# wiedenhoeft/HaMMLET

Hardware: AMD Instinct MI355X
Metric: block-updates/sec (Gibbs sweep) + HBM GB/s, 10^8 pos / 5 states (higher is better)
Workload: dtype f32; 1 GPU; c3_1e8_k5_dynamic; positions=100000000, states=5, block_structure=dynamic, chains=1, parallelism=chain-parallel x1

## Files before the change

hammlet_amd/csrc/hml_capi.hip:

```cpp
#include "hml_capi_shared.hpp"

static thread_local std::string g_err;
int hml_set_err(int code, const std::string& msg) { g_err = msg; return code; }

static const hml_ktab* ktab(int K);
#define HML_KTAB(KV, tab) const hml_ktab* tab = ktab(KV); if (!tab) return set_err(HML_ERR_ARG, "number of states must be in [2,16]")

std::atomic<int> hml_live_ctx[64];
int hml_ctx_bind(hml_ctx* c) { return ctx_bind(c); }
int hml_ctx_fetch_model(hml_ctx* c, hml_model* out) { return fetch_model(c, out); }

HML_KERNEL void hml_k_debug_eval(int fn, const float* __restrict__ a, const float* __restrict__ b, float* __restrict__ out,
                                 uint64_t n, uint64_t seed) {
    if (fn == 24) {
        const uint64_t nw = ((uint64_t)gridDim.x * blockDim.x) >> 6;
        if ((threadIdx.x & 63) != 0) return;
        for (uint64_t i = ((uint64_t)blockIdx.x * blockDim.x + threadIdx.x) >> 6; i < n; i += nw) {
            hml_dev_src src;
            src.s = hml_stream_open(hml_make_key(seed, 0), HML_KIND_THETA, seed, (uint32_t)i);
            out[i] = hml_gamma_f32<hml_devmath>(src, a[i], b[i]);
        }
        return;
    }
    const uint64_t stride = (uint64_t)gridDim.x * blockDim.x;
    for (uint64_t i = (uint64_t)blockIdx.x * blockDim.x + threadIdx.x; i < n; i += stride) {
        const float x = a[i], y = b ? b[i] : 0.0f;
        float r = 0.0f;
        switch (fn) {
            case 0: r = hml_expf(x); break;
            case 1: r = hml_logf(x); break;
            case 2: r = hml_powf_unit(x, y); break;
            case 3: r = HML_SQRTF(x); break;
            case 4: r = x / y; break;
            case 5: {
                hml_dev_src src;
                src.s = hml_stream_open(hml_make_key(seed, 0), HML_KIND_THETA, seed, (uint32_t)i);
                r = hml_gamma_f32<hml_devmath>(src, x, y);
            } break;
            case 6: {
                hml_dev_src src;
                src.s = hml_stream_open(hml_make_key(seed, 0), HML_KIND_PI, seed, (uint32_t)i);
                hml_normal_f32<hml_devmath> nd;
                r = nd.draw(src, x, y);
            } break;
            case 7: r = (float)hml_log((double)x); break;
            case 8: r = (float)hml_exp_nonpos((double)x); break;
            case 9: r = (float)((double)x / (double)y); break;
            case 40: r = hml_glibc_expf(x); break;
            case 41: r = hml_glibc_logf(x); break;
            case 42: r = hml_glibc_powf_unit(x, y); break;
            case 43: { const double Zd = (double)y; r = hml_tr2_quotient(x, Zd, hml_tr2_reciprocal(Zd)); } break;
            case 10: r = (float)(1.0 / (double)x); break;
            case 12: case 13: case 14: case 15: case 16: case 17: case 18: case 19: case 20: case 21: case 22: case 23: {
                hml_dev_src src; src.s = hml_stream_open(hml_make_key(seed, 0), HML_KIND_THETA, seed, (uint32_t)i);
                const float alpha = x, beta = y; (void)beta;
                const float malpha = alpha < 1.0f ? alpha + 1.0f : alpha;
                const float a1 = malpha - 1.0f / 3.0f;
                const float a2 = 1.0f / hml_devmath::sqrtf_(9.0f * a1);
                hml_normal_f32<hml_devmath> nd;
                float n = nd.draw(src, 0.0f, 1.0f);
                float v = 1.0f + a2 * n;
                float v3 = v * v * v;
                float u = hml_canonical_f32(src);
                const bool c1 = (double)u > (double)1.0f - 0.0331 * (double)n * (double)n * (double)n * (double)n;
                const bool c2 = ((double)hml_devmath::logf_(u) > (0.5 * (double)n * (double)n + (double)a1 * ((1.0 - (double)v3) + (double)hml_devmath::logf_(v3))));
                float n2 = nd.draw(src, 0.0f, 1.0f);
                float vb = 1.0f + a2 * n2;
                float vb3 = vb * vb * vb;
                float ub = hml_canonical_f32(src);
                const bool d1 = (double)ub > (double)1.0f - 0.0331 * (double)n2 * (double)n2 * (double)n2 * (double)n2;
                const bool d2 = ((double)hml_devmath::logf_(ub) > (0.5 * (double)n2 * (double)n2 + (double)a1 * ((1.0 - (double)vb3) + (double)hml_devmath::logf_(vb3))));
                r = fn == 12 ? n : fn == 13 ? v3 : fn == 14 ? u : fn == 15 ? (float)(c1 ? 1 : 0) + 2.0f * (c2 ? 1 : 0) : fn == 16 ? n2 : fn == 17 ? a2
                    : fn == 18 ? vb3 : fn == 19 ? ub : fn == 20 ? (float)(d1 ? 1 : 0) + 2.0f * (d2 ? 1 : 0) : fn == 21 ? (float)src.s.n : 0.0f;
                if (fn == 22) r = nd.draw(src, 0.0f, 1.0f);
                if (fn == 23) { hml_normal_f32<hml_devmath> nf; r = nf.draw(src, 0.0f, 1.0f); r = nf.draw(src, 0.0f, 1.0f); }
            } break;
            case 30: case 31: {
                r = 0.0f;
                const int Kc = fn == 30 ? 16 : 5;
                if (i % Kc == 0 && i + Kc <= n) {
                    bool unsure = false;
                    int fastr, lit;
                    if (fn == 30) { float w[16]; for (int j = 0; j < 16; ++j) w[j] = a[i + j]; fastr = hml_categorical_k_fast<16>(w, (double)y, unsure); lit = hml_categorical_k_literal<16>(w, (double)y); if (unsure) fastr = lit; }
                    else { float w[5]; for (int j = 0; j < 5; ++j) w[j] = a[i + j]; fastr = hml_categorical_k_fast<5>(w, (double)y, unsure); lit = hml_categorical_k_literal<5>(w, (double)y); if (unsure) fastr = lit; }
                    out[i] = (float)fastr; out[i + 1] = (float)lit; out[i + 2] = unsure ? 1.0f : 0.0f;
                }
                continue;
            }
            case 11: { const double d = HML_SQRT((double)x * 1.0000001); r = (float)((d - (double)(float)d) * 1e9); } break;
        }
        out[i] = r;
    }
}

static bool parse_band_edges(const char* text, int* n, float* edges) {
    *n = 0;
    const char* p = text;
    while (*p) {
        char* end = nullptr;
        const float v = strtof(p, &end);
        if (end == p || *n >= HML_MAX_BAND_EDGES) return false;
        edges[(*n)++] = v;
        p = end;
// ... 1121 lines not shown
        for (int k = 0; k < n; ++k) {
            hml_ctx* c = cs[k];
            if (int r = ctx_bind(c)) return r;
            if (record && c->rec_marginals && c->pooled) return set_err(HML_ERR_ARG, "the marginals of a context are pooled (common labels, several chains): further sweeps cannot be recorded into them");
            if (chain_halted(c)) { if (int r = hml_settle(c)) return r; }
            log_sweep(c, method, record);
            if (int r = sweep_dispatch(c, method, record)) return r;
            if (record && c->cb) {
                HIPCHK(hipStreamSynchronize(c->stream));
                if (chain_halted(c)) { if (int r = hml_settle(c)) return r; continue; }
                if (int r = check_device_error(c)) return r;
                c->cb(c, i, c->cb_user);
            }
        }
    }
    return 0;
}

extern "C" {

int hml_set_option(hml_ctx* c, const char* name, int value) {
    if (!c || !name) return set_err(HML_ERR_ARG, "null argument");
    if (std::string(name) == "weight_keys") {
        if (c->loaded) return set_err(HML_ERR_ARG, "weight_keys must be set before the observations are loaded");
        c->use_keys = value != 0;
        c->summary_always = value == 2;
        return 0;
    }
    if (std::string(name) == "max_blocks") {
        if (c->loaded) return set_err(HML_ERR_ARG, "max_blocks must be set before the observations are loaded");
        if (value < 0) return set_err(HML_ERR_ARG, "max_blocks: a number of blocks, or 0 for the default");
        c->cap_opt = (uint64_t)value;
        return 0;
    }
    if (std::string(name) == "fused_blocks") {
        c->fused_blocks = value != 0;
        c->fused_keep = value == 2;
        if (c->graph_exec) { hipGraphExecDestroy(c->graph_exec); c->graph_exec = nullptr; }
        return 0;
    }
    if (std::string(name) == "compat") {
        if (c->model_set) return set_err(HML_ERR_ARG, "compat must be set before the model");
        c->compat = value != 0;
        return 0;
    }
    if (std::string(name) == "trellis_L") {
        if (value < 0 || value > HML_TRE_MAX_L || value % 32) return set_err(HML_ERR_ARG, "trellis_L: 0 or a multiple of 32 up to 1024");
        c->tre_L = (uint32_t)value;
        return 0;
    }
    return set_err(HML_ERR_ARG, std::string("unknown option ") + name);
}

int hml_sync(hml_ctx* c) {
    if (!c) return set_err(HML_ERR_ARG, "null context");
    if (int r = ctx_bind(c)) return r;
    if (int r = hml_settle(c)) return r;
    if (c->d_dbg && getenv("HML_FUSED_DEBUG") && atoi(getenv("HML_FUSED_DEBUG")) == 2) {
        std::vector<unsigned long long> h(4096 * 8);
        hipMemcpy(h.data(), c->d_dbg, h.size() * 8, hipMemcpyDeviceToHost);
        uint32_t n = 0; while (n < 4096 && h[n * 8]) ++n;
        unsigned long long t0 = ~0ull; for (uint32_t i = 0; i < n; ++i) t0 = std::min(t0, h[i * 8]);
        double mx[5] = {0, 0, 0, 0, 0}, av[5] = {0, 0, 0, 0, 0};
        if (n) for (uint32_t i = 0; i < n; ++i) for (int k = 0; k < 5; ++k) { const double d = (double)(h[i * 8 + k] - t0) * 0.01; mx[k] = std::max(mx[k], d); av[k] += d / n; }
        if (n) fprintf(stderr, "[fused-many dbg] n=%u start avg %.2f max %.2f | phaseA avg %.2f max %.2f | requested avg %.2f max %.2f | offsets avg %.2f max %.2f | end avg %.2f max %.2f (us)\n",
                n, av[0], mx[0], av[1], mx[1], av[2], mx[2], av[3], mx[3], av[4], mx[4]);
        if (n) for (uint32_t i : {0u, n / 4, n / 2, n - 1}) if (i < n) fprintf(stderr, "   wg %u: %.2f %.2f %.2f %.2f %.2f | wavefront 0: parameters in LDS %.2f, weights arrived %.2f, its lists done %.2f\n", i, (h[i*8]-t0)*0.01, (h[i*8+1]-t0)*0.01, (h[i*8+2]-t0)*0.01, (h[i*8+3]-t0)*0.01, (h[i*8+4]-t0)*0.01,
                                                                                  (h[i*8+5]-t0)*0.01, (h[i*8+6]-t0)*0.01, (h[i*8+7]-t0)*0.01);
    } else if (c->d_dbg) {
        std::vector<unsigned long long> h(4096 * 4);
        hipMemcpy(h.data(), c->d_dbg, h.size() * 8, hipMemcpyDeviceToHost);
        const uint32_t n = (uint32_t)std::min<uint64_t>(4096, (c->T + HML_FUSED_SUB_POSITIONS - 1) / HML_FUSED_SUB_POSITIONS);
        unsigned long long t0 = ~0ull; for (uint32_t i = 0; i < n; ++i) if (h[i * 4]) t0 = std::min(t0, h[i * 4]);
        double mx[4] = {0, 0, 0, 0}, av[4] = {0, 0, 0, 0};
        for (uint32_t i = 0; i < n; ++i) for (int k = 0; k < 4; ++k) { const double d = (double)(h[i * 4 + k] - t0) * 0.01; mx[k] = std::max(mx[k], d); av[k] += d / n; }
        fprintf(stderr, "[fused dbg] n=%u start avg %.2f max %.2f | phaseA avg %.2f max %.2f | offsets avg %.2f max %.2f | end avg %.2f max %.2f (us)\n", n, av[0], mx[0], av[1], mx[1], av[2], mx[2], av[3], mx[3]);
        { uint32_t late = 0, first_late = n; for (uint32_t i = 0; i < n; ++i) if ((h[i * 4] - t0) * 0.01 > 2.0) { ++late; first_late = std::min(first_late, i); }
          fprintf(stderr, "   late starters: %u, first index %u\n", late, first_late); }
        for (uint32_t i : {0u, n / 4, n / 2, n - 1}) fprintf(stderr, "   wg %u: %.2f %.2f %.2f %.2f\n", i, (h[i*4]-t0)*0.01, (h[i*4+1]-t0)*0.01, (h[i*4+2]-t0)*0.01, (h[i*4+3]-t0)*0.01);
    }
    if (c->model_set && getenv("HML_PARAMS_DEBUG")) {
        hml_model m;
        if (fetch_model(c, &m) == 0) {
            fprintf(stderr, "[params dbg] us since the kernel's start: accumulators read %.2f | tree %.2f | theta drawn %.2f | A gammas %.2f | barrier %.2f | end %.2f\n",
                    (m.dbg_t[1] - m.dbg_t[0]) * 0.01, (m.dbg_t[2] - m.dbg_t[0]) * 0.01, (m.dbg_t[3] - m.dbg_t[0]) * 0.01, (m.dbg_t[4] - m.dbg_t[0]) * 0.01,
                    (m.dbg_t[5] - m.dbg_t[0]) * 0.01, (m.dbg_t[6] - m.dbg_t[0]) * 0.01);
            fprintf(stderr, "[params dbg]   theta's gamma core + normal drawn %.2f | last wavefront's tree %.2f\n", (m.dbg_t[7] - m.dbg_t[0]) * 0.01, (m.dbg_t[8] - m.dbg_t[0]) * 0.01);
        }
    }
    if (c->model_set) return check_device_error(c);
    return 0;
}


static int current_B(hml_ctx* c, uint32_t* B) {
    HIPCHK(hipMemcpyAsync(c->h_B, &c->d_mdl->B, sizeof(uint32_t), hipMemcpyDeviceToHost, c->stream));
    HIPCHK(hipStreamSynchronize(c->stream));
    *B = *c->h_B;
    return 0;
}

int hml_get_num_blocks(hml_ctx* c, uint64_t* B) {
    NEED_LOADED();
    uint32_t b; if (int r = current_B(c, &b)) return r;
    *B = b; return 0;
}
int hml_get_blocks(hml_ctx* c, uint32_t* starts) {
    NEED_LOADED();
    uint32_t b; if (int r = current_B(c, &b)) return r;
    HIPCHK(hipMemcpy(starts, c->d_starts, ((uint64_t)b + 1) * sizeof(uint32_t), hipMemcpyDeviceToHost));
    return 0;
}
int hml_get_block_stats(hml_ctx* c, float* sum, float* sum_sq) {
    NEED_LOADED();
    uint32_t b; if (int r = current_B(c, &b)) return r;
    std::vector<float2> v(b);
    for (int d = 0; d < c->D; ++d) {
        HIPCHK(hipMemcpy(v.data(), c->d_bstat + (uint64_t)d * c->T, (uint64_t)b * sizeof(float2), hipMemcpyDeviceToHost));
        for (uint32_t i = 0; i < b; ++i) { sum[(uint64_t)d * b + i] = v[i].x; sum_sq[(uint64_t)d * b + i] = v[i].y; }
    }
    return 0;
}
int hml_get_states(hml_ctx* c, int16_t* q) {
    NEED_MODEL();
    uint32_t b; if (int r = current_B(c, &b)) return r;
    HIPCHK(hipMemcpy(q, c->d_q, (uint64_t)b * sizeof(int16_t), hipMemcpyDeviceToHost));
    return 0;
}
int hml_get_theta(hml_ctx* c, float* mean_var) {
    NEED_MODEL();
    hml_model m; if (int r = fetch_model(c, &m)) return r;
    for (int k = 0; k < m.P; ++k) { mean_var[2 * k] = m.mu[k]; mean_var[2 * k + 1] = m.var[k]; }
    return 0;
}
int hml_get_dimensions(hml_ctx* c, int* D, int* P) {
    if (!c) return set_err(HML_ERR_ARG, "null context");
    if (D) *D = c->D;
    if (P) *P = c->P > 0 ? c->P : c->K;
    return 0;
}
int hml_get_transitions(hml_ctx* c, float* A, float* pi) {
    NEED_MODEL();
    hml_model m; if (int r = fetch_model(c, &m)) return r;
    if (A) memcpy(A, m.A, (size_t)c->K * c->K * sizeof(float));
    if (pi) memcpy(pi, m.pi, (size_t)c->K * sizeof(float));
    return 0;
}
int hml_set_parameters(hml_ctx* c, const float* mean_var, const float* A, const float* pi) {
    NEED_MODEL();
    hml_model m; if (int r = fetch_model(c, &m)) return r;
    const int K = c->K;
    for (int k = 0; k < m.P; ++k) {
        const float mean = mean_var[2 * k], var = mean_var[2 * k + 1];
        if (!std::isfinite(mean)) return set_err(HML_ERR_MODEL, "Mean (" + std::to_string(mean) + ") must be set to a finite value!");
        if (!std::isfinite(var)) return set_err(HML_ERR_MODEL, "Variance(" + std::to_string(var) + ") must be set to a finite value!");
        if (var <= 0) return set_err(HML_ERR_MODEL, "Variance (" + std::to_string(var) + ") must be positive!");
        m.mu[k] = mean; m.var[k] = var; m.sd[k] = sqrtf(var);
    }
    memcpy(m.A, A, (size_t)K * K * sizeof(float));
    memcpy(m.pi, pi, (size_t)K * sizeof(float));
    HIPCHK(hipMemcpyAsync(c->d_mdl, &m, sizeof m, hipMemcpyHostToDevice, c->stream));
    if (c->compat) hipLaunchKernelGGL(hml_k_compat_derive, dim3(1), dim3(64), 0, c->stream, c->d_mdl);
    else if (c->wide) hipLaunchKernelGGL(hml_k_wide_derive, dim3(1), dim3(64), 0, c->stream, c->d_mdl);
    else { HML_KTAB(K, kt); kt->derive(c); }
    KLAUNCH_CHECK();
    HIPCHK(hipStreamSynchronize(c->stream));
    if (c->dynamic) c->blocks_valid = false;
    return 0;
}
int hml_get_threshold(hml_ctx* c, float* thr) {
// ... 164 lines not shown
```

hammlet_amd/csrc/hml_k_params.h:

```cpp
#ifndef HML_K_PARAMS_H
#define HML_K_PARAMS_H

#include <type_traits>

#include "hml_dist.h"
#include "hml_k_backward.h"
#include "hml_state.h"

struct hml_dev_src {
    hml_stream s;
    __device__ __forceinline__ uint32_t next() { return hml_stream_next(&s); }
};

template <int K>
__device__ __forceinline__ void hml_derive(hml_model* mdl, int tid) {
    const int P = mdl->P, D = mdl->D;
    if (tid < P) {
        const float m = mdl->mu[tid], v = mdl->var[tid], sd = mdl->sd[tid];
        mdl->logN[tid] = hml_logf(sd) + m * m / (2 * v);
        mdl->rvar2[tid] = 1.0 / (2.0 * (double)v);
    }
    if (tid < K) {
        float r = 0.0f;
        for (int d = 0; d < D; ++d) {
            const int pp = mdl->map[tid][d];
            const float m = mdl->mu[pp], v = mdl->var[pp], sd = mdl->sd[pp];
            r += hml_logf(sd) + m * m / (2 * v);
        }
        mdl->logNs[tid] = r;
        mdl->logA[tid] = hml_logf(mdl->A[tid * K + tid]);
    }
    if (tid == 0) {
        float mv = HML_INF_F;
        for (int k = 0; k < P; ++k) { const float v = mdl->var[k]; mv = (v < mv) ? v : mv; }
        const float l = hml_logf((float)mdl->T);
        const float arg = 2 * l * mv;
        const float t = HML_SQRTF(arg);
        mdl->thr_theta = t;
        if (mdl->dynamic) mdl->thr = t;
    }
}

template <int K>
HML_KERNEL __launch_bounds__(64) void hml_k_derive(hml_model* mdl) { hml_derive<K>(mdl, threadIdx.x); }

HML_KERNEL __launch_bounds__(64) void hml_k_set_dynamic(hml_model* mdl, int on, int take_threshold) {
    if (threadIdx.x == 0) {
        mdl->dynamic = on;
        if (take_threshold) mdl->thr = mdl->thr_theta;
    }
}

template <int K, bool SPREAD, bool MANY = false>
__device__ __forceinline__ void hml_b_params(hml_model* __restrict__ mdl, typename std::conditional<SPREAD, double, const double>::type* __restrict__ partial,
                                                     int mode, int leaf, int nleaf) {
    __shared__ double wp[16][K][2];
    __shared__ uint32_t s_last;
    __shared__ float fin[K][2];
    __shared__ float graw[K * K];
    __shared__ float praw[K];
    __shared__ unsigned long long s_trans[K * K];
    __shared__ unsigned long long s_occ[K];
    const int tid = threadIdx.x, lane = tid & 63, wave = tid >> 6;
    if (mode == 0 && mdl->halted != 0u) return;
    if (tid == 0) mdl->dbg_t[0] = wall_clock64();
    __shared__ float s_var[K], s_logN[K];
    const int P = mdl->P, D = mdl->D;
    const unsigned long long epoch = mdl->epoch;
    const hml_key key = mdl->key;
    float hyp0 = 0.0f, hyp1 = 0.0f, hyp2 = 0.0f, hyp3 = 0.0f;
    if (wave == 0 && lane < P) { hyp0 = mdl->nig_post[lane][0]; hyp1 = mdl->nig_post[lane][1]; hyp2 = mdl->nig_post[lane][2]; hyp3 = mdl->nig_post[lane][3]; }
    if (wave == 1 && lane < K) hyp0 = mdl->dirPi[lane];
    if (tid >= 128 && tid < 128 + K * K) hyp0 = mdl->dirA[tid - 128];
    unsigned long long acc_total = 0ull;
    if (tid >= 128 && tid < 128 + K * K) {
        const int e = tid - 128;
        unsigned long long v[HML_CNT_SPLIT];
#pragma unroll
        for (int sp = 0; sp < HML_CNT_SPLIT; ++sp) v[sp] = mdl->trans[sp][e];
        unsigned long long t = 0ull;
#pragma unroll
        for (int sp = 0; sp < HML_CNT_SPLIT; ++sp) { t += v[sp]; if (!SPREAD) mdl->trans[sp][e] = 0ull; }
        s_trans[e] = t;
        if (!SPREAD) mdl->last_trans[e] = t;
        acc_total = t;
    }
    if (tid >= 512 && tid < 512 + K) {
        const int k = tid - 512;
        unsigned long long v[HML_CNT_SPLIT];
#pragma unroll
        for (int sp = 0; sp < HML_CNT_SPLIT; ++sp) v[sp] = mdl->occ[sp][k];
        unsigned long long t = 0ull;
#pragma unroll
        for (int sp = 0; sp < HML_CNT_SPLIT; ++sp) { t += v[sp]; if (!SPREAD) mdl->occ[sp][k] = 0ull; }
        s_occ[k] = t;
        if (!SPREAD) mdl->last_occ[k] = t;
        acc_total = t;
    }
    typename std::conditional<SPREAD, double, const double>::type* const level1 = partial + (uint64_t)HML_REDUCE_GROUPS * 2 * K;
    if constexpr (SPREAD) {
        for (int idx = wave; idx < 2 * K; idx += 16) {
            const double r = hml_wave_tree_f64(partial[(uint64_t)idx * HML_REDUCE_GROUPS + 64u * (uint32_t)leaf + (uint32_t)lane]);
            if (lane == 0) __hip_atomic_store(reinterpret_cast<unsigned long long*>(level1) + leaf * 2 * K + idx, hml_d2u(r), __ATOMIC_RELAXED, __HIP_MEMORY_SCOPE_AGENT);
        }
    }
    constexpr int NDRAW = 2 + (K * K + 63) / 64;
    static_assert(2 * NDRAW <= 16, "wavefronts of the parameter kernel");
    const bool draws = wave < NDRAW;
    const int mirror = wave - (16 - NDRAW);
    double part_s[K], part_q[K], part2_s[K], part2_q[K];
#pragma unroll
    for (int s = 0; s < K; ++s) {
        part_s[s] = (!SPREAD && mode == 0 && !draws) ? partial[(uint64_t)(s * 2 + 0) * HML_REDUCE_GROUPS + tid] : 0.0;
        part_q[s] = (!SPREAD && mode == 0 && !draws) ? partial[(uint64_t)(s * 2 + 1) * HML_REDUCE_GROUPS + tid] : 0.0;
        part2_s[s] = (!SPREAD && mode == 0 && mirror >= 0) ? partial[(uint64_t)(s * 2 + 0) * HML_REDUCE_GROUPS + (mirror * 64 + lane)] : 0.0;
        part2_q[s] = (!SPREAD && mode == 0 && mirror >= 0) ? partial[(uint64_t)(s * 2 + 1) * HML_REDUCE_GROUPS + (mirror * 64 + lane)] : 0.0;
    }

    if (SPREAD) __syncthreads();
    else asm volatile("s_waitcnt lgkmcnt(0)\n\ts_barrier" ::: "memory");
    if (tid == 0) mdl->dbg_t[1] = wall_clock64();
    if constexpr (SPREAD) {
        static_assert(NDRAW <= 8, "wavefronts 8 (occupancies) and 15 (ticket) draw nothing");
        if (wave == 15) {
            uint32_t last = 0u;
            if (lane == 0) {
                __threadfence();
                const uint32_t t = atomicAdd(&mdl->params_ticket, 1u);
                last = ((t + 1u) % (uint32_t)nleaf == 0u) ? 1u : 0u;
                s_last = last;
            }
            last = (uint32_t)__builtin_amdgcn_readfirstlane((int)last);
            if (last != 0u) {
                __threadfence();
                if (lane < 2 * K) {
                    unsigned long long raw[16];
#pragma unroll
                    for (int i = 0; i < 16; ++i) raw[i] = __hip_atomic_load(reinterpret_cast<unsigned long long*>(level1) + i * 2 * K + lane, __ATOMIC_RELAXED, __HIP_MEMORY_SCOPE_AGENT);
#pragma unroll
                    for (int i = 0; i < 16; ++i) wp[i][lane >> 1][lane & 1] = hml_u2d(raw[i]);
                }
            }
        }
    }

    unsigned long long cnt = 0ull;
    float th_alpha = hyp0, th_gcore = 0.0f, th_z = 0.0f;
    if (wave == 0 && lane < P) {
        const int k = lane;
        if (mode == 0) {
            if (D == 1) cnt = s_occ[k];
            else for (int st = 0; st < K; ++st) for (int d = 0; d < D; ++d) if (mdl->map[st][d] == k) cnt += s_occ[st];
        }
        if (cnt > 0ull) th_alpha = (float)((double)hyp0 + (double)cnt / 2.0);
        hml_dev_src src;
        src.s = hml_stream_open(key, HML_KIND_THETA, epoch, (uint32_t)k);
        th_gcore = hml_gamma_core_f32<hml_devmath>(src, th_alpha);
        hml_normal_f32<hml_devmath> nd;
        th_z = nd.draw_std(src);
        if (tid == 0) mdl->dbg_t[7] = wall_clock64();
    }
    if (mode != 2) {
        if (wave == 1 && lane < K) {
            const int k = lane;
            const float al = hyp0 + (float)s_occ[k];
            hml_dev_src src;
            src.s = hml_stream_open(key, HML_KIND_PI, epoch, (uint32_t)k);
            praw[k] = hml_gamma_f32<hml_devmath>(src, al, 1.0f);
        }
        if (tid >= 128 && tid < 128 + K * K) {
            const int e = tid - 128;
            const float al = hyp0 + (float)s_trans[e];
            hml_dev_src src;
            src.s = hml_stream_open(key, HML_KIND_TRANS, epoch, (uint32_t)e);
            graw[e] = hml_gamma_f32<hml_devmath>(src, al, 1.0f);
        }
    }
    if (tid == 128) mdl->dbg_t[4] = wall_clock64();

    if constexpr (SPREAD) {
        __syncthreads();
        if (s_last == 0u) return;
        if (tid >= 128 && tid < 128 + K * K) {
            const int e = tid - 128;
#pragma unroll
            for (int sp = 0; sp < HML_CNT_SPLIT; ++sp) mdl->trans[sp][e] = 0ull;
            mdl->last_trans[e] = acc_total;
        }
        if (tid >= 512 && tid < 512 + K) {
            const int k = tid - 512;
#pragma unroll
            for (int sp = 0; sp < HML_CNT_SPLIT; ++sp) mdl->occ[sp][k] = 0ull;
            mdl->last_occ[k] = acc_total;
        }
    }
    if (mode == 0) {
        if (!SPREAD && !draws) {
#pragma unroll
            for (int s = 0; s < K; ++s) {
                const double a = hml_wave_tree_f64(part_s[s]), d = hml_wave_tree_f64(part_q[s]);
                if (lane == 0) { wp[wave][s][0] = a; wp[wave][s][1] = d; }
            }
        }
        if (!SPREAD && mirror >= 0) {
#pragma unroll
            for (int s = 0; s < K; ++s) {
                const double a = hml_wave_tree_f64(part2_s[s]), d = hml_wave_tree_f64(part2_q[s]);
                if (lane == 0) { wp[mirror][s][0] = a; wp[mirror][s][1] = d; }
            }
        }
        if (tid == 1023) mdl->dbg_t[8] = wall_clock64();
        __syncthreads();
        if (tid < 2 * K) {
            const int s = tid >> 1, c = tid & 1;
            double v[16];
#pragma unroll
            for (int i = 0; i < 16; ++i) v[i] = wp[i][s][c];
#pragma unroll
            for (int st = 1; st < 16; st <<= 1)
#pragma unroll
                for (int i = 0; i < 16; i += 2 * st) v[i] = v[i] + v[i + st];
            fin[s][c] = (float)v[0];
        }
        __syncthreads();
        if (tid == 0) mdl->dbg_t[2] = wall_clock64();
    }

    if (wave == 0 && lane < P) {
        const int k = lane;
        float alpha = hyp0, beta = hyp1, mu0 = hyp2, nu = hyp3;
        if (mode == 0) { mdl->last_sum[k] = fin[k][0]; mdl->last_sumsq[k] = fin[k][1]; }
        if (cnt > 0ull) {
            const float sum = fin[k][0], sumSq = fin[k][1];
            if (sumSq < 0.0f) hml_raise(mdl, HML_DEVERR_NEG_SUMSQ, sumSq);
            const double N = (double)cnt;
            const float xbar = (float)((double)sum / N);
            float ssN = (float)((double)(sum * sum) / N);
            if (ssN > sumSq) ssN = sumSq;
            const float na = th_alpha;
            const float dxm = (xbar - mu0) * (xbar - mu0);
            const float nb = (float)((double)beta +
                                     (((double)sumSq + (N * (double)nu / (N + (double)nu)) * (double)dxm) - (double)ssN) / 2.0);
            const float nm = (float)((double)(nu * mu0 + sum) / ((double)nu + N));
            const float nn = (float)((double)nu + N);
            if (na <= 0.0f) hml_raise(mdl, HML_DEVERR_NIG_ALPHA, na);
            if (nb <= 0.0f) hml_raise(mdl, HML_DEVERR_NIG_BETA, nb);
            if (nn <= 0.0f) hml_raise(mdl, HML_DEVERR_NIG_NU, nn);
            if (!hml_isfinite(nm)) hml_raise(mdl, HML_DEVERR_NIG_MU0, nm);
            alpha = na; beta = nb; mu0 = nm; nu = nn;
        }
        (void)alpha;
        const float g = th_gcore * (float)(1.0 / (double)beta);
        const float v = (float)(1.0 / (double)g);
        const float m = th_z * HML_SQRTF(v / nu) + mu0;
        if (!hml_isfinite(m)) hml_raise(mdl, HML_DEVERR_MEAN_NOT_FINITE, m);
        if (!hml_isfinite(v)) hml_raise(mdl, HML_DEVERR_VAR_NOT_FINITE, v);
        else if (v <= 0.0f) hml_raise(mdl, HML_DEVERR_VAR_NOT_POSITIVE, v);
        const float sd = HML_SQRTF(v);
        mdl->mu[k] = m; mdl->var[k] = v; mdl->sd[k] = sd;
        mdl->rvar2[k] = 1.0 / (2.0 * (double)v);
        if (mode == 0) {
            const float ln = hml_logf(sd) + m * m / (2 * v);
            mdl->logN[k] = ln;
            s_logN[k] = ln;
            s_var[k] = v;
        }
#pragma unroll
        for (int i = 0; i < 4; ++i) mdl->nig_post[k][i] = mdl->nig_prior[i];
        if (tid == 0) mdl->dbg_t[3] = wall_clock64();
    }
    __syncthreads();
    if (tid == 0) mdl->dbg_t[5] = wall_clock64();
    if (mode != 2) {
        if (tid < K) {
            float sum = 0.0f;
#pragma unroll
            for (int d = 0; d < K; ++d) sum += graw[tid * K + d];
#pragma unroll
            for (int d = 0; d < K; ++d) mdl->A[tid * K + d] = graw[tid * K + d] / sum;
            if (mode == 0) {
                mdl->logA[tid] = hml_logf(graw[tid * K + tid] / sum);
                float r = 0.0f;
                for (int d = 0; d < D; ++d) r += s_logN[mdl->map[tid][d]];
                mdl->logNs[tid] = r;
            }
        }
        if (mode == 0 && tid == 65) {
            float mv = HML_INF_F;
#pragma unroll
            for (int k = 0; k < P; ++k) { const float v = s_var[k]; mv = (v < mv) ? v : mv; }
            const float l = hml_logf((float)mdl->T);
            const float arg = 2 * l * mv;
            const float t = HML_SQRTF(arg);
            mdl->thr_theta = t;
            if (mdl->dynamic) mdl->thr = t;
        }
        if (tid == 64) {
            float sum = 0.0f;
#pragma unroll
            for (int d = 0; d < K; ++d) sum += praw[d];
#pragma unroll
            for (int d = 0; d < K; ++d) mdl->pi[d] = praw[d] / sum;
        }
        if (tid >= 128 && tid < 128 + K * K) {
            const int e = tid - 128;
            mdl->dirA[e] = (e / K == e % K) ? mdl->a_diag : mdl->a_off;
        }
        if (tid >= 512 && tid < 512 + K) {
            const int k = tid - 512;
            mdl->dirPi[k] = mdl->pi_alpha;
        }
    }
    if (mode != 0) {
        __threadfence_block();
        __syncthreads();
        hml_derive<K>(mdl, tid);
    }
    if (tid == 1023) {
        if (mode == 0) {
            uint32_t W = mdl->fwd_W;
            const unsigned long long refits = mdl->forward_refits - mdl->fwd_refits_seen;
            const unsigned long long serial = mdl->forward_serial - mdl->fwd_serial_seen;
            const unsigned long long handful = (mdl->B >> 22) ? (((unsigned long long)(mdl->B >> 16) > 16ull) ? (unsigned long long)(mdl->B >> 16) : 16ull) : 0ull;
            if (mdl->tre_fused && (mdl->B >> 22)) {
                const unsigned long long hi = (unsigned long long)(mdl->B >> mdl->tre_hi_shift) + 16ull, lo = (unsigned long long)(mdl->B >> mdl->tre_lo_shift) + 2ull;
                if (serial != 0ull || refits > hi) {
                    W = (W + 8u < (uint32_t)HML_TRE_HALO_MAX) ? W + 8u : (uint32_t)HML_TRE_HALO_MAX;
                    mdl->tre_W_floor = W;
                    mdl->tre_floor_age = 0u;
                } else {
                    if (++mdl->tre_floor_age >= 256u) { mdl->tre_floor_age = 0u; mdl->tre_W_floor = (mdl->tre_W_floor > 8u) ? mdl->tre_W_floor - 8u : 0u; }
                    const uint32_t lowest = (mdl->tre_W_floor > 8u) ? mdl->tre_W_floor : 8u;
                    if (refits < lo && W >= lowest + 8u) W -= 8u;
                }
                if (W > (uint32_t)HML_TRE_HALO_MAX) W = (uint32_t)HML_TRE_HALO_MAX;
            } else
            {
            if (mdl->wl_W_need != 0u && ++mdl->wl_need_age > 128u) mdl->wl_W_need = 0u;
            if (serial != 0ull || refits > handful) {
                if (mdl->sweeps >= (unsigned long long)mdl->fwd_burnin_sweeps && (serial != 0ull || refits >= 16ull) && !MANY) { mdl->wl_W_need = W; mdl->wl_need_age = 0u; }
                W = (2u * W < 1024u) ? 2u * W : 1024u; mdl->fwd_quiet = 0u;
            } else if (refits == 0ull) {
                uint32_t floorW = (mdl->sweeps < (unsigned long long)mdl->fwd_burnin_sweeps) ? mdl->fwd_W_burnin : mdl->fwd_W0;
                if (mdl->wl_W_need != 0u) { const uint32_t keep = ((mdl->wl_W_need + 8u) & ~7u) < 1024u ? ((mdl->wl_W_need + 8u) & ~7u) : 1024u; floorW = keep > floorW ? keep : floorW; }
                if (++mdl->fwd_quiet >= mdl->fwd_quiet_need) {
                    const uint32_t w2 = W - W / 4u;
                    const uint32_t lower = (w2 > floorW) ? ((w2 & ~7u) > floorW ? (w2 & ~7u) : floorW) : floorW;
                    W = lower < W ? lower : W;
                    mdl->fwd_quiet = 0u;
                }
            } else mdl->fwd_quiet = 0u;
            }
            mdl->fwd_W = W;
            mdl->fwd_refits_seen = mdl->forward_refits;
            mdl->fwd_serial_seen = mdl->forward_serial;
            mdl->fwd_serial_ran = 0u;
        }
        mdl->dbg_t[6] = wall_clock64();
        mdl->fwd_mismatch = 0u;
        mdl->fwd_mismatch2 = 0u;
        mdl->epoch = epoch + 1ull;
        if (mode == 0) { mdl->sweeps += 1ull; mdl->block_updates += (unsigned long long)mdl->B; }
    }
}
template <int K>
HML_KERNEL __launch_bounds__(1024) void hml_k_params(hml_model* __restrict__ mdl, const double* __restrict__ partial,
                                                     int mode) {
    hml_b_params<K, false>(mdl, partial, mode, 0, 1);
}
#define HML_PARAMS_TREE_WGS 16
template <int K>
HML_KERNEL __launch_bounds__(1024) void hml_k_params_spread(hml_model* __restrict__ mdl, double* __restrict__ partial) {
    hml_b_params<K, true>(mdl, partial, 0, (int)blockIdx.x, (int)gridDim.x);
}


#endif
```

Before: 3.085 billion block-updates/s.

## Precompute RNG word table in LDS and hoist all model loads in params kernel

The parameter kernel now issues every global read it needs (hyperparameters, count accumulators, adaptation state, reduction partials) up front, before the halt check. It then fills a shared-memory table with the first 16 random words for each theta, pi and transition variate, with all threads working in parallel. The gamma and normal draws are spread across rows in several wavefronts and read the table, falling back to the stream generator only when more words are needed. The adaptation bookkeeping reads preloaded lane values through readlane instead of reloading from global memory, aiming to shorten the latency-bound serial path of this small kernel, at the cost of more LDS, more registers and more complex code.

New measurement: 3.101 billion block-updates/s, median of 5. About the same (+0.5%).

```diff
diff --git a/hammlet_amd/csrc/hml_capi.hip b/hammlet_amd/csrc/hml_capi.hip
--- a/hammlet_amd/csrc/hml_capi.hip
+++ b/hammlet_amd/csrc/hml_capi.hip
@@ -19,6 +19,44 @@
             hml_dev_src src;
             src.s = hml_stream_open(hml_make_key(seed, 0), HML_KIND_THETA, seed, (uint32_t)i);
             out[i] = hml_gamma_f32<hml_devmath>(src, a[i], b[i]);
+        }
+        return;
+    }
+    if (fn >= 25 && fn <= 29) {
+        __shared__ __attribute__((aligned(16))) uint32_t tab[256][HML_PTAB_WORDS];
+        if (blockDim.x > 256u) return;
+        uint32_t* const row = tab[threadIdx.x];
+        const hml_key key = hml_make_key(seed, 0);
+        uint64_t first = (uint64_t)blockIdx.x * blockDim.x + threadIdx.x, step = (uint64_t)gridDim.x * blockDim.x;
+        if (fn == 29) {
+            if ((threadIdx.x & 63) != 0) return;
+            first >>= 6; step >>= 6;
+        }
+        for (uint64_t i = first; i < n; i += step) {
+            if ((fn == 27 || fn == 28) && ((i & 1u) != 0u || i + 1 >= n)) continue;
+            const int blocks = (fn == 26) ? 1 : HML_PTAB_WORDS / 4;
+            if (fn != 28) for (int blk = 0; blk < blocks; ++blk) hml_tab_fill_pair(row, key, HML_KIND_THETA, seed, (uint32_t)i, (uint32_t)blk);
+            if (fn == 26) {
+                hml_tab_src<4> src;
+                src.open(row, key, HML_KIND_THETA, seed, (uint32_t)i);
+                out[i] = hml_gamma_f32<hml_devmath>(src, a[i], b[i]);
+            } else if (fn == 27) {
+                hml_tab_src<HML_PTAB_WORDS> src;
+                src.open(row, key, HML_KIND_THETA, seed, (uint32_t)i);
+                out[i] = hml_gamma_core_f32<hml_devmath>(src, a[i]);
+                hml_normal_f32<hml_devmath> nd;
+                out[i + 1] = nd.draw_std(src);
+            } else if (fn == 28) {
+                hml_dev_src src;
+                src.s = hml_stream_open(key, HML_KIND_THETA, seed, (uint32_t)i);
+                out[i] = hml_gamma_core_f32<hml_devmath>(src, a[i]);
+                hml_normal_f32<hml_devmath> nd;
+                out[i + 1] = nd.draw_std(src);
+            } else {
+                hml_tab_src<HML_PTAB_WORDS> src;
+                src.open(row, key, HML_KIND_THETA, seed, (uint32_t)i);
+                out[i] = hml_gamma_f32<hml_devmath>(src, a[i], b[i]);
+            }
         }
         return;
     }
@@ -1306,10 +1344,11 @@
     if (c->model_set && getenv("HML_PARAMS_DEBUG")) {
         hml_model m;
         if (fetch_model(c, &m) == 0) {
-            fprintf(stderr, "[params dbg] us since the kernel's start: accumulators read %.2f | tree %.2f | theta drawn %.2f | A gammas %.2f | barrier %.2f | end %.2f\n",
+            fprintf(stderr, "[params dbg] us since the kernel's entry: first barrier (accumulators read, word table filled) %.2f | tree %.2f | theta drawn %.2f | A gammas %.2f | barrier %.2f | end %.2f\n",
                     (m.dbg_t[1] - m.dbg_t[0]) * 0.01, (m.dbg_t[2] - m.dbg_t[0]) * 0.01, (m.dbg_t[3] - m.dbg_t[0]) * 0.01, (m.dbg_t[4] - m.dbg_t[0]) * 0.01,
                     (m.dbg_t[5] - m.dbg_t[0]) * 0.01, (m.dbg_t[6] - m.dbg_t[0]) * 0.01);
-            fprintf(stderr, "[params dbg]   theta's gamma core + normal drawn %.2f | last wavefront's tree %.2f\n", (m.dbg_t[7] - m.dbg_t[0]) * 0.01, (m.dbg_t[8] - m.dbg_t[0]) * 0.01);
+            fprintf(stderr, "[params dbg]   word table filled %.2f | theta's gamma core + normal drawn %.2f | last wavefront's tree %.2f\n", (m.dbg_t[9] - m.dbg_t[0]) * 0.01,
+                    (m.dbg_t[7] - m.dbg_t[0]) * 0.01, (m.dbg_t[8] - m.dbg_t[0]) * 0.01);
         }
     }
     if (c->model_set) return check_device_error(c);
diff --git a/hammlet_amd/csrc/hml_k_params.h b/hammlet_amd/csrc/hml_k_params.h
--- a/hammlet_amd/csrc/hml_k_params.h
+++ b/hammlet_amd/csrc/hml_k_params.h
@@ -10,6 +10,41 @@
 struct hml_dev_src {
     hml_stream s;
     __device__ __forceinline__ uint32_t next() { return hml_stream_next(&s); }
+};
+
+#define HML_PTAB_WORDS 16
+template <int K> struct hml_ptab {
+    static constexpr int ROWS = 2 * K + K * K;
+    __device__ static __forceinline__ uint32_t kind(int r) { return r < K ? (uint32_t)HML_KIND_THETA : r < 2 * K ? (uint32_t)HML_KIND_PI : (uint32_t)HML_KIND_TRANS; }
+    __device__ static __forceinline__ uint32_t index(int r) { return (uint32_t)(r < K ? r : r < 2 * K ? r - K : r - 2 * K); }
+};
+__device__ __forceinline__ void hml_tab_fill_pair(uint32_t* row, hml_key key, uint32_t kind, uint64_t epoch, uint32_t index, uint32_t block) {
+    const hml_u32x4 o = hml_stream4(key, kind, epoch, index, block);
+    row[4 * block + 0] = o.v[0]; row[4 * block + 1] = o.v[1]; row[4 * block + 2] = o.v[2]; row[4 * block + 3] = o.v[3];
+}
+static __device__ __noinline__ hml_u32x4 hml_tab_block_beyond(uint32_t k0, uint32_t k1, uint32_t kind, uint32_t epoch_lo, uint32_t epoch_hi, uint32_t index, uint32_t draw4) {
+    hml_key key; key.k0 = k0; key.k1 = k1;
+    return hml_stream4(key, kind, ((uint64_t)epoch_hi << 32) | (uint64_t)epoch_lo, index, draw4);
+}
+template <int NT>
+struct hml_tab_src {
+    static_assert(NT % 4 == 0 && NT <= HML_PTAB_WORDS, "the table ends on a block boundary");
+    const uint32_t* row;
+    hml_key key;
+    uint32_t kind, index, n;
+    uint64_t epoch;
+    hml_u32x4 buf;
+    __device__ __forceinline__ void open(const uint32_t* row_, hml_key key_, uint32_t kind_, uint64_t epoch_, uint32_t index_) {
+        row = row_; key = key_; kind = kind_; epoch = epoch_; index = index_; n = 0u;
+        buf.v[0] = buf.v[1] = buf.v[2] = buf.v[3] = 0u;
+    }
+    __device__ __forceinline__ uint32_t next() {
+        const uint32_t i = n++;
+        if (i < (uint32_t)NT) return row[i];
+        const uint32_t l = i & 3u;
+        if (l == 0u) buf = hml_tab_block_beyond(key.k0, key.k1, kind, (uint32_t)epoch, (uint32_t)(epoch >> 32), index, i >> 2);
+        return l == 0u ? buf.v[0] : l == 1u ? buf.v[1] : l == 2u ? buf.v[2] : buf.v[3];
+    }
 };
 
 template <int K>
@@ -61,53 +96,68 @@
     __shared__ float praw[K];
     __shared__ unsigned long long s_trans[K * K];
     __shared__ unsigned long long s_occ[K];
-    const int tid = threadIdx.x, lane = tid & 63, wave = tid >> 6;
-    if (mode == 0 && mdl->halted != 0u) return;
-    if (tid == 0) mdl->dbg_t[0] = wall_clock64();
+    __shared__ __attribute__((aligned(16))) uint32_t s_tab[hml_ptab<K>::ROWS][HML_PTAB_WORDS];
+    __shared__ float s_thg[K], s_thz[K], s_tha[K];
+    __shared__ unsigned long long s_thn[K];
     __shared__ float s_var[K], s_logN[K];
+    const int tid = threadIdx.x, lane = tid & 63, wave = __builtin_amdgcn_readfirstlane(tid >> 6);
+    constexpr int ROWS = hml_ptab<K>::ROWS;
+    constexpr int NDRAW = SPREAD ? 8 : ((ROWS + 63) / 64 > 4 ? (ROWS + 63) / 64 : 4);
+    static_assert(2 * NDRAW <= 16, "wavefronts of the parameter kernel");
+    static_assert((ROWS + NDRAW - 1) / NDRAW <= 64, "variates of one wavefront");
+    const bool draws = wave < NDRAW;
+    const int mirror = wave - (16 - NDRAW);
+    const int row = lane * NDRAW + wave;
+    const bool has_row = draws && row < ROWS;
+    const bool is_theta = has_row && row < K, is_pi = has_row && row >= K && row < 2 * K, is_tr = has_row && row >= 2 * K;
+
+    const uint32_t halted = mdl->halted;
     const int P = mdl->P, D = mdl->D;
     const unsigned long long epoch = mdl->epoch;
     const hml_key key = mdl->key;
-    float hyp0 = 0.0f, hyp1 = 0.0f, hyp2 = 0.0f, hyp3 = 0.0f;
-    if (wave == 0 && lane < P) { hyp0 = mdl->nig_post[lane][0]; hyp1 = mdl->nig_post[lane][1]; hyp2 = mdl->nig_post[lane][2]; hyp3 = mdl->nig_post[lane][3]; }
-    if (wave == 1 && lane < K) hyp0 = mdl->dirPi[lane];
-    if (tid >= 128 && tid < 128 + K * K) hyp0 = mdl->dirA[tid - 128];
-    unsigned long long acc_total = 0ull;
-    if (tid >= 128 && tid < 128 + K * K) {
-        const int e = tid - 128;
-        unsigned long long v[HML_CNT_SPLIT];
-#pragma unroll
-        for (int sp = 0; sp < HML_CNT_SPLIT; ++sp) v[sp] = mdl->trans[sp][e];
-        unsigned long long t = 0ull;
-#pragma unroll
-        for (int sp = 0; sp < HML_CNT_SPLIT; ++sp) { t += v[sp]; if (!SPREAD) mdl->trans[sp][e] = 0ull; }
-        s_trans[e] = t;
-        if (!SPREAD) mdl->last_trans[e] = t;
-        acc_total = t;
-    }
-    if (tid >= 512 && tid < 512 + K) {
-        const int k = tid - 512;
-        unsigned long long v[HML_CNT_SPLIT];
-#pragma unroll
-        for (int sp = 0; sp < HML_CNT_SPLIT; ++sp) v[sp] = mdl->occ[sp][k];
-        unsigned long long t = 0ull;
-#pragma unroll
-        for (int sp = 0; sp < HML_CNT_SPLIT; ++sp) { t += v[sp]; if (!SPREAD) mdl->occ[sp][k] = 0ull; }
-        s_occ[k] = t;
-        if (!SPREAD) mdl->last_occ[k] = t;
-        acc_total = t;
+    const float h_nig_prior0 = mdl->nig_prior[0], h_nig_prior1 = mdl->nig_prior[1], h_nig_prior2 = mdl->nig_prior[2], h_nig_prior3 = mdl->nig_prior[3];
+    const float h_a_off = mdl->a_off, h_a_diag = mdl->a_diag, h_pi_alpha = mdl->pi_alpha;
+    const uint32_t h_T = mdl->T;
+    const int32_t h_dynamic = mdl->dynamic;
+    const unsigned long long t_entry = wall_clock64();
+    const uint32_t hyp_off = is_theta ? (uint32_t)offsetof(hml_model, nig_post) + 16u * (uint32_t)row
+                             : is_pi  ? (uint32_t)offsetof(hml_model, dirPi) + 4u * (uint32_t)(row - K)
+                             : is_tr  ? (uint32_t)offsetof(hml_model, dirA) + 4u * (uint32_t)(row - 2 * K)
+                                      : (uint32_t)offsetof(hml_model, nig_post);
+    const float hyp0 = *reinterpret_cast<const float*>(reinterpret_cast<const char*>(mdl) + hyp_off);
+    const float* const nig_at = mdl->nig_post[tid < K ? tid : 0];
+    const float nig0 = nig_at[0], nig1 = nig_at[1], nig2 = nig_at[2], nig3 = nig_at[3];
+    constexpr uint32_t ADAPT_AT = (uint32_t)offsetof(hml_model, fwd_mismatch), ADAPT_WORDS = ((uint32_t)offsetof(hml_model, params_ticket) - ADAPT_AT) / 4u;
+    constexpr uint32_t COUNT_AT = (uint32_t)offsetof(hml_model, epoch), COUNT_WORDS = ((uint32_t)offsetof(hml_model, n_recorded) - COUNT_AT) / 4u;
+    static_assert(ADAPT_WORDS <= 64u && COUNT_WORDS <= 64u, "a word a lane");
+    uint32_t adapt_w = 0u, count_w = 0u, other_w = 0u;
+    if (wave == 15) {
+        const char* const base = reinterpret_cast<const char*>(mdl);
+        adapt_w = *reinterpret_cast<const uint32_t*>(base + ADAPT_AT + 4u * ((uint32_t)lane < ADAPT_WORDS ? (uint32_t)lane : 0u));
+        count_w = *reinterpret_cast<const uint32_t*>(base + COUNT_AT + 4u * ((uint32_t)lane < COUNT_WORDS ? (uint32_t)lane : 0u));
+        other_w = *reinterpret_cast<const uint32_t*>(base + (lane == 1 ? (uint32_t)offsetof(hml_model, wl_W_need) : lane == 2 ? (uint32_t)offsetof(hml_model, wl_need_age) : (uint32_t)offsetof(hml_model, B)));
+    }
+    constexpr int TRW = (K * K + 63) / 64;
+    static_assert(2 + TRW <= 8, "wavefront 8 gathers the occupancies");
+    unsigned long long acc[HML_CNT_SPLIT];
+#pragma unroll
+    for (int sp = 0; sp < HML_CNT_SPLIT; ++sp) acc[sp] = 0ull;
+    if (wave >= 2 && wave < 2 + TRW) {
+        const int e = (tid - 128 < K * K) ? tid - 128 : K * K - 1;
+#pragma unroll
+        for (int sp = 0; sp < HML_CNT_SPLIT; ++sp) acc[sp] = mdl->trans[sp][e];
+    }
+    if (wave == 8) {
+        const int k = (tid - 512 < K) ? tid - 512 : K - 1;
+#pragma unroll
+        for (int sp = 0; sp < HML_CNT_SPLIT; ++sp) acc[sp] = mdl->occ[sp][k];
     }
     typename std::conditional<SPREAD, double, const double>::type* const level1 = partial + (uint64_t)HML_REDUCE_GROUPS * 2 * K;
+    double lvl_a = 0.0, lvl_b = 0.0;
     if constexpr (SPREAD) {
-        for (int idx = wave; idx < 2 * K; idx += 16) {
-            const double r = hml_wave_tree_f64(partial[(uint64_t)idx * HML_REDUCE_GROUPS + 64u * (uint32_t)leaf + (uint32_t)lane]);
-            if (lane == 0) __hip_atomic_store(reinterpret_cast<unsigned long long*>(level1) + leaf * 2 * K + idx, hml_d2u(r), __ATOMIC_RELAXED, __HIP_MEMORY_SCOPE_AGENT);
-        }
-    }
-    constexpr int NDRAW = 2 + (K * K + 63) / 64;
-    static_assert(2 * NDRAW <= 16, "wavefronts of the parameter kernel");
-    const bool draws = wave < NDRAW;
-    const int mirror = wave - (16 - NDRAW);
+        if (wave < 2 * K) lvl_a = partial[(uint64_t)wave * HML_REDUCE_GROUPS + 64u * (uint32_t)leaf + (uint32_t)lane];
+        if (wave + 16 < 2 * K) lvl_b = partial[(uint64_t)(wave + 16) * HML_REDUCE_GROUPS + 64u * (uint32_t)leaf + (uint32_t)lane];
+    }
     double part_s[K], part_q[K], part2_s[K], part2_q[K];
 #pragma unroll
     for (int s = 0; s < K; ++s) {
@@ -115,6 +165,50 @@
         part_q[s] = (!SPREAD && mode == 0 && !draws) ? partial[(uint64_t)(s * 2 + 1) * HML_REDUCE_GROUPS + tid] : 0.0;
         part2_s[s] = (!SPREAD && mode == 0 && mirror >= 0) ? partial[(uint64_t)(s * 2 + 0) * HML_REDUCE_GROUPS + (mirror * 64 + lane)] : 0.0;
         part2_q[s] = (!SPREAD && mode == 0 && mirror >= 0) ? partial[(uint64_t)(s * 2 + 1) * HML_REDUCE_GROUPS + (mirror * 64 + lane)] : 0.0;
+    }
+    asm volatile("" ::: "memory");
+
+    if (mode == 0 && halted != 0u) return;
+    if (tid == 0) mdl->dbg_t[0] = t_entry;
+
+#pragma unroll
+    for (int p0 = 0; p0 < 4 * ROWS; p0 += 1024) {
+        const int p = p0 + tid;
+        if (p < 4 * ROWS) {
+            const int r = p >> 2;
+            hml_tab_fill_pair(s_tab[r], key, hml_ptab<K>::kind(r), epoch, hml_ptab<K>::index(r), (uint32_t)(p & 3));
+        }
+    }
+    if (tid == 0) mdl->dbg_t[9] = wall_clock64();
+
+    unsigned long long acc_total = 0ull;
+    if (tid >= 128 && tid < 128 + K * K) {
+        const int e = tid - 128;
+        unsigned long long t = 0ull;
+#pragma unroll
+        for (int sp = 0; sp < HML_CNT_SPLIT; ++sp) { t += acc[sp]; if (!SPREAD) mdl->trans[sp][e] = 0ull; }
+        s_trans[e] = t;
+        if (!SPREAD) mdl->last_trans[e] = t;
+        acc_total = t;
+    }
+    if (tid >= 512 && tid < 512 + K) {
+        const int k = tid - 512;
+        unsigned long long t = 0ull;
+#pragma unroll
+        for (int sp = 0; sp < HML_CNT_SPLIT; ++sp) { t += acc[sp]; if (!SPREAD) mdl->occ[sp][k] = 0ull; }
+        s_occ[k] = t;
+        if (!SPREAD) mdl->last_occ[k] = t;
+        acc_total = t;
+    }
+    if constexpr (SPREAD) {
+        if (wave < 2 * K) {
+            const double r = hml_wave_tree_f64(lvl_a);
+            if (lane == 0) __hip_atomic_store(reinterpret_cast<unsigned long long*>(level1) + leaf * 2 * K + wave, hml_d2u(r), __ATOMIC_RELAXED, __HIP_MEMORY_SCOPE_AGENT);
+        }
+        if (wave + 16 < 2 * K) {
+            const double r = hml_wave_tree_f64(lvl_b);
+            if (lane == 0) __hip_atomic_store(reinterpret_cast<unsigned long long*>(level1) + leaf * 2 * K + wave + 16, hml_d2u(r), __ATOMIC_RELAXED, __HIP_MEMORY_SCOPE_AGENT);
+        }
     }
 
     if (SPREAD) __syncthreads();
@@ -144,36 +238,30 @@
         }
     }
 
-    unsigned long long cnt = 0ull;
-    float th_alpha = hyp0, th_gcore = 0.0f, th_z = 0.0f;
-    if (wave == 0 && lane < P) {
-        const int k = lane;
-        if (mode == 0) {
-            if (D == 1) cnt = s_occ[k];
-            else for (int st = 0; st < K; ++st) for (int d = 0; d < D; ++d) if (mdl->map[st][d] == k) cnt += s_occ[st];
-        }
-        if (cnt > 0ull) th_alpha = (float)((double)hyp0 + (double)cnt / 2.0);
-        hml_dev_src src;
-        src.s = hml_stream_open(key, HML_KIND_THETA, epoch, (uint32_t)k);
-        th_gcore = hml_gamma_core_f32<hml_devmath>(src, th_alpha);
-        hml_normal_f32<hml_devmath> nd;
-        th_z = nd.draw_std(src);
-        if (tid == 0) mdl->dbg_t[7] = wall_clock64();
-    }
-    if (mode != 2) {
-        if (wave == 1 && lane < K) {
-            const int k = lane;
-            const float al = hyp0 + (float)s_occ[k];
-            hml_dev_src src;
-            src.s = hml_stream_open(key, HML_KIND_PI, epoch, (uint32_t)k);
-            praw[k] = hml_gamma_f32<hml_devmath>(src, al, 1.0f);
-        }
-        if (tid >= 128 && tid < 128 + K * K) {
-            const int e = tid - 128;
-            const float al = hyp0 + (float)s_trans[e];
-            hml_dev_src src;
-            src.s = hml_stream_open(key, HML_KIND_TRANS, epoch, (uint32_t)e);
-            graw[e] = hml_gamma_f32<hml_devmath>(src, al, 1.0f);
+    {
+        const bool th = is_theta && row < P, dir = (is_pi || is_tr) && mode != 2;
+        if (th || dir) {
+            unsigned long long cnt = 0ull;
+            float alpha = hyp0;
+            if (th) {
+                const int k = row;
+                if (mode == 0) {
+                    if (D == 1) cnt = s_occ[k];
+                    else for (int st = 0; st < K; ++st) for (int d = 0; d < D; ++d) if (mdl->map[st][d] == k) cnt += s_occ[st];
+                }
+                if (cnt > 0ull) alpha = (float)((double)hyp0 + (double)cnt / 2.0);
+            } else if (is_pi) alpha = hyp0 + (float)s_occ[row - K];
+            else alpha = hyp0 + (float)s_trans[row - 2 * K];
+            hml_tab_src<HML_PTAB_WORDS> src;
+            src.open(s_tab[row], key, hml_ptab<K>::kind(row), epoch, hml_ptab<K>::index(row));
+            const float g = hml_gamma_core_f32<hml_devmath>(src, alpha);
+            if (th) {
+                hml_normal_f32<hml_devmath> nd;
+                const float z = nd.draw_std(src);
+                s_thg[row] = g; s_thz[row] = z; s_tha[row] = alpha; s_thn[row] = cnt;
+                if (tid == 0) mdl->dbg_t[7] = wall_clock64();
+            } else if (is_pi) praw[row - K] = g * 1.0f;
+            else graw[row - 2 * K] = g * 1.0f;
         }
     }
     if (tid == 128) mdl->dbg_t[4] = wall_clock64();
@@ -226,9 +314,12 @@
         if (tid == 0) mdl->dbg_t[2] = wall_clock64();
     }
 
-    if (wave == 0 && lane < P) {
-        const int k = lane;
-        float alpha = hyp0, beta = hyp1, mu0 = hyp2, nu = hyp3;
+    if (mode != 0 && !SPREAD) __syncthreads();
+    if (tid < K && tid < P) {
+        const int k = tid;
+        float alpha = nig0, beta = nig1, mu0 = nig2, nu = nig3;
+        const unsigned long long cnt = s_thn[k];
+        const float th_alpha = s_tha[k], th_gcore = s_thg[k], th_z = s_thz[k];
         if (mode == 0) { mdl->last_sum[k] = fin[k][0]; mdl->last_sumsq[k] = fin[k][1]; }
         if (cnt > 0ull) {
             const float sum = fin[k][0], sumSq = fin[k][1];
@@ -265,35 +356,36 @@
             s_logN[k] = ln;
             s_var[k] = v;
         }
-#pragma unroll
-        for (int i = 0; i < 4; ++i) mdl->nig_post[k][i] = mdl->nig_prior[i];
+        mdl->nig_post[k][0] = h_nig_prior0; mdl->nig_post[k][1] = h_nig_prior1; mdl->nig_post[k][2] = h_nig_prior2; mdl->nig_post[k][3] = h_nig_prior3;
         if (tid == 0) mdl->dbg_t[3] = wall_clock64();
     }
     __syncthreads();
     if (tid == 0) mdl->dbg_t[5] = wall_clock64();
     if (mode != 2) {
-        if (tid < K) {
+        if (tid < K * K) {
+            const int i = tid / K;
             float sum = 0.0f;
 #pragma unroll
-            for (int d = 0; d < K; ++d) sum += graw[tid * K + d];
-#pragma unroll
-            for (int d = 0; d < K; ++d) mdl->A[tid * K + d] = graw[tid * K + d] / sum;
-            if (mode == 0) {
-                mdl->logA[tid] = hml_logf(graw[tid * K + tid] / sum);
-                float r = 0.0f;
-                for (int d = 0; d < D; ++d) r += s_logN[mdl->map[tid][d]];
-                mdl->logNs[tid] = r;
-            }
+            for (int d = 0; d < K; ++d) sum += graw[i * K + d];
+            const float q = graw[tid] / sum;
+            mdl->A[tid] = q;
+            if (mode == 0 && tid == i * K + i) mdl->logA[i] = hml_logf(q);
+        }
+        if (mode == 0 && tid >= 256 && tid < 256 + K) {
+            const int k = tid - 256;
+            float r = 0.0f;
+            for (int d = 0; d < D; ++d) r += s_logN[mdl->map[k][d]];
+            mdl->logNs[k] = r;
         }
         if (mode == 0 && tid == 65) {
             float mv = HML_INF_F;
 #pragma unroll
             for (int k = 0; k < P; ++k) { const float v = s_var[k]; mv = (v < mv) ? v : mv; }
-            const float l = hml_logf((float)mdl->T);
+            const float l = hml_logf((float)h_T);
             const float arg = 2 * l * mv;
             const float t = HML_SQRTF(arg);
             mdl->thr_theta = t;
-            if (mdl->dynamic) mdl->thr = t;
+            if (h_dynamic) mdl->thr = t;
         }
         if (tid == 64) {
             float sum = 0.0f;
@@ -304,11 +396,11 @@
         }
         if (tid >= 128 && tid < 128 + K * K) {
             const int e = tid - 128;
-            mdl->dirA[e] = (e / K == e % K) ? mdl->a_diag : mdl->a_off;
+            mdl->dirA[e] = (e / K == e % K) ? h_a_diag : h_a_off;
         }
         if (tid >= 512 && tid < 512 + K) {
             const int k = tid - 512;
-            mdl->dirPi[k] = mdl->pi_alpha;
+            mdl->dirPi[k] = h_pi_alpha;
         }
     }
     if (mode != 0) {
@@ -316,51 +408,78 @@
         __syncthreads();
         hml_derive<K>(mdl, tid);
     }
+#define HML_ADAPT32(field) ((uint32_t)__builtin_amdgcn_readlane((int)adapt_w, (int)(((uint32_t)offsetof(hml_model, field) - ADAPT_AT) / 4u)))
+#define HML_ADAPT64(field) ((unsigned long long)(uint32_t)__builtin_amdgcn_readlane((int)adapt_w, (int)(((uint32_t)offsetof(hml_model, field) - ADAPT_AT) / 4u)) | \
+                            ((unsigned long long)(uint32_t)__builtin_amdgcn_readlane((int)adapt_w, (int)(((uint32_t)offsetof(hml_model, field) - ADAPT_AT) / 4u + 1u)) << 32))
+#define HML_COUNT64(field) ((unsigned long long)(uint32_t)__builtin_amdgcn_readlane((int)count_w, (int)(((uint32_t)offsetof(hml_model, field) - COUNT_AT) / 4u)) | \
+                            ((unsigned long long)(uint32_t)__builtin_amdgcn_readlane((int)count_w, (int)(((uint32_t)offsetof(hml_model, field) - COUNT_AT) / 4u + 1u)) << 32))
+    uint32_t h_B = 0u, h_fwd_W = 0u, h_fwd_W0 = 0u, h_fwd_quiet = 0u, h_fwd_W_burnin = 0u, h_fwd_burnin_sweeps = 0u, h_fwd_quiet_need = 0u;
+    uint32_t h_tre_fused = 0u, h_tre_hi_shift = 0u, h_tre_lo_shift = 0u, h_tre_W_floor = 0u, h_tre_floor_age = 0u, h_wl_W_need = 0u, h_wl_need_age = 0u;
+    unsigned long long h_forward_refits = 0ull, h_forward_serial = 0ull, h_fwd_refits_seen = 0ull, h_fwd_serial_seen = 0ull, h_sweeps = 0ull, h_block_updates = 0ull;
+    if (wave == 15) {
+        h_B = (uint32_t)__builtin_amdgcn_readlane((int)other_w, 0);
+        h_wl_W_need = (uint32_t)__builtin_amdgcn_readlane((int)other_w, 1);
+        h_wl_need_age = (uint32_t)__builtin_amdgcn_readlane((int)other_w, 2);
+        h_fwd_W = HML_ADAPT32(fwd_W); h_fwd_W0 = HML_ADAPT32(fwd_W0); h_fwd_quiet = HML_ADAPT32(fwd_quiet); h_fwd_W_burnin = HML_ADAPT32(fwd_W_burnin);
+        h_fwd_burnin_sweeps = HML_ADAPT32(fwd_burnin_sweeps); h_fwd_quiet_need = HML_ADAPT32(fwd_quiet_need);
+        h_tre_fused = HML_ADAPT32(tre_fused); h_tre_hi_shift = HML_ADAPT32(tre_hi_shift); h_tre_lo_shift = HML_ADAPT32(tre_lo_shift);
+        h_tre_W_floor = HML_ADAPT32(tre_W_floor); h_tre_floor_age = HML_ADAPT32(tre_floor_age);
+        h_fwd_refits_seen = HML_ADAPT64(fwd_refits_seen); h_fwd_serial_seen = HML_ADAPT64(fwd_serial_seen);
+        h_forward_refits = HML_COUNT64(forward_refits); h_forward_serial = HML_COUNT64(forward_serial);
+        h_sweeps = HML_COUNT64(sweeps); h_block_updates = HML_COUNT64(block_updates);
+    }
+#undef HML_ADAPT32
+#undef HML_ADAPT64
+#undef HML_COUNT64
     if (tid == 1023) {
         if (mode == 0) {
-            uint32_t W = mdl->fwd_W;
-            const unsigned long long refits = mdl->forward_refits - mdl->fwd_refits_seen;
-            const unsigned long long serial = mdl->forward_serial - mdl->fwd_serial_seen;
-            const unsigned long long handful = (mdl->B >> 22) ? (((unsigned long long)(mdl->B >> 16) > 16ull) ? (unsigned long long)(mdl->B >> 16) : 16ull) : 0ull;
-            if (mdl->tre_fused && (mdl->B >> 22)) {
-                const unsigned long long hi = (unsigned long long)(mdl->B >> mdl->tre_hi_shift) + 16ull, lo = (unsigned long long)(mdl->B >> mdl->tre_lo_shift) + 2ull;
+            uint32_t W = h_fwd_W;
+            const unsigned long long refits = h_forward_refits - h_fwd_refits_seen;
+            const unsigned long long serial = h_forward_serial - h_fwd_serial_seen;
+            const unsigned long long handful = (h_B >> 22) ? (((unsigned long long)(h_B >> 16) > 16ull) ? (unsigned long long)(h_B >> 16) : 16ull) : 0ull;
+            if (h_tre_fused && (h_B >> 22)) {
+                uint32_t W_floor = h_tre_W_floor, floor_age = h_tre_floor_age;
+                const unsigned long long hi = (unsigned long long)(h_B >> h_tre_hi_shift) + 16ull, lo = (unsigned long long)(h_B >> h_tre_lo_shift) + 2ull;
                 if (serial != 0ull || refits > hi) {
                     W = (W + 8u < (uint32_t)HML_TRE_HALO_MAX) ? W + 8u : (uint32_t)HML_TRE_HALO_MAX;
-                    mdl->tre_W_floor = W;
-                    mdl->tre_floor_age = 0u;
+                    W_floor = W;
+                    floor_age = 0u;
                 } else {
-                    if (++mdl->tre_floor_age >= 256u) { mdl->tre_floor_age = 0u; mdl->tre_W_floor = (mdl->tre_W_floor > 8u) ? mdl->tre_W_floor - 8u : 0u; }
-                    const uint32_t lowest = (mdl->tre_W_floor > 8u) ? mdl->tre_W_floor : 8u;
+                    if (++floor_age >= 256u) { floor_age = 0u; W_floor = (W_floor > 8u) ? W_floor - 8u : 0u; }
+                    const uint32_t lowest = (W_floor > 8u) ? W_floor : 8u;
                     if (refits < lo && W >= lowest + 8u) W -= 8u;
                 }
                 if (W > (uint32_t)HML_TRE_HALO_MAX) W = (uint32_t)HML_TRE_HALO_MAX;
+                mdl->tre_W_floor = W_floor; mdl->tre_floor_age = floor_age;
             } else
             {
-            if (mdl->wl_W_need != 0u && ++mdl->wl_need_age > 128u) mdl->wl_W_need = 0u;
+            uint32_t W_need = h_wl_W_need, need_age = h_wl_need_age, quiet = h_fwd_quiet;
+            if (W_need != 0u && ++need_age > 128u) W_need = 0u;
             if (serial != 0ull || refits > handful) {
-                if (mdl->sweeps >= (unsigned long long)mdl->fwd_burnin_sweeps && (serial != 0ull || refits >= 16ull) && !MANY) { mdl->wl_W_need = W; mdl->wl_need_age = 0u; }
-                W = (2u * W < 1024u) ? 2u * W : 1024u; mdl->fwd_quiet = 0u;
+                if (h_sweeps >= (unsigned long long)h_fwd_burnin_sweeps && (serial != 0ull || refits >= 16ull) && !MANY) { W_need = W; need_age = 0u; }
+                W = (2u * W < 1024u) ? 2u * W : 1024u; quiet = 0u;
             } else if (refits == 0ull) {
-                uint32_t floorW = (mdl->sweeps < (unsigned long long)mdl->fwd_burnin_sweeps) ? mdl->fwd_W_burnin : mdl->fwd_W0;
-                if (mdl->wl_W_need != 0u) { const uint32_t keep = ((mdl->wl_W_need + 8u) & ~7u) < 1024u ? ((mdl->wl_W_need + 8u) & ~7u) : 1024u; floorW = keep > floorW ? keep : floorW; }
-                if (++mdl->fwd_quiet >= mdl->fwd_quiet_need) {
+                uint32_t floorW = (h_sweeps < (unsigned long long)h_fwd_burnin_sweeps) ? h_fwd_W_burnin : h_fwd_W0;
+                if (W_need != 0u) { const uint32_t keep = ((W_need + 8u) & ~7u) < 1024u ? ((W_need + 8u) & ~7u) : 1024u; floorW = keep > floorW ? keep : floorW; }
+                if (++quiet >= h_fwd_quiet_need) {
                     const uint32_t w2 = W - W / 4u;
                     const uint32_t lower = (w2 > floorW) ? ((w2 & ~7u) > floorW ? (w2 & ~7u) : floorW) : floorW;
                     W = lower < W ? lower : W;
-                    mdl->fwd_quiet = 0u;
+                    quiet = 0u;
                 }
-            } else mdl->fwd_quiet = 0u;
+            } else quiet = 0u;
+            mdl->wl_W_need = W_need; mdl->wl_need_age = need_age; mdl->fwd_quiet = quiet;
             }
             mdl->fwd_W = W;
-            mdl->fwd_refits_seen = mdl->forward_refits;
-            mdl->fwd_serial_seen = mdl->forward_serial;
+            mdl->fwd_refits_seen = h_forward_refits;
+            mdl->fwd_serial_seen = h_forward_serial;
             mdl->fwd_serial_ran = 0u;
         }
         mdl->dbg_t[6] = wall_clock64();
         mdl->fwd_mismatch = 0u;
         mdl->fwd_mismatch2 = 0u;
         mdl->epoch = epoch + 1ull;
-        if (mode == 0) { mdl->sweeps += 1ull; mdl->block_updates += (unsigned long long)mdl->B; }
+        if (mode == 0) { mdl->sweeps = h_sweeps + 1ull; mdl->block_updates = h_block_updates + (unsigned long long)h_B; }
     }
 }
 template <int K>
```
